# avaneev/avir

Measured on NVIDIA H100. Metric: Mpixels/sec resize (8K->4K RGBA), higher is better.
Workload: dtype f32

## Files before the change

avir_b200/csrc/stream_chain.cu:

```cuda
#include <cuda.h>
#include <cuda_runtime.h>

#include "stream_kernel.cuh"
#include "stream_launch.h"

#if !defined(AVS_CHAIN_ID) || !defined(AVS_CHAIN_PASS)
#error "compile with -DAVS_CHAIN_ID=<StreamChainId> -DAVS_CHAIN_PASS=<0 row pass | 1 column pass>"
#endif

namespace avs {

namespace {

typedef CUresult (*EncodeTiledFn)(CUtensorMap*, CUtensorMapDataType, cuuint32_t, void*, const cuuint64_t*,
                                  const cuuint64_t*, const cuuint32_t*, const cuuint32_t*, CUtensorMapInterleave,
                                  CUtensorMapSwizzle, CUtensorMapL2promotion, CUtensorMapFloatOOBfill);
EncodeTiledFn encode_tiled() {
    static const EncodeTiledFn fn = [] {
        void* f = nullptr;
        cudaDriverEntryPointQueryResult q;
        if (cudaGetDriverEntryPoint("cuTensorMapEncodeTiled", &f, cudaEnableDefault, &q) != cudaSuccess ||
            q != cudaDriverEntryPointSuccess)
            f = nullptr;
        return reinterpret_cast<EncodeTiledFn>(f);
    }();
    return fn;
}

bool encode_source_tensor(StreamParams& p, int box_rows) {
    static_assert(sizeof(CUtensorMap) == sizeof(p.tmap), "tensor map size");
    EncodeTiledFn enc = encode_tiled();
    if (!enc) return false;
    const cuuint64_t dims[2] = {(cuuint64_t)p.n_lines * 4, (cuuint64_t)(p.src_len - p.src_row_base)};
    const cuuint64_t strides[1] = {(cuuint64_t)p.src_pitch * 4};
    const cuuint32_t box[2] = {64, (cuuint32_t)box_rows};
    const cuuint32_t estr[2] = {1, 1};
    if (dims[1] < 1) return false;
    return enc(reinterpret_cast<CUtensorMap*>(p.tmap), CU_TENSOR_MAP_DATA_TYPE_FLOAT32, 2, const_cast<void*>(p.src),
               dims, strides, box, estr, CU_TENSOR_MAP_INTERLEAVE_NONE, CU_TENSOR_MAP_SWIZZLE_NONE,
               CU_TENSOR_MAP_L2_PROMOTION_L2_256B, CU_TENSOR_MAP_FLOAT_OOB_FILL_NONE) == CUDA_SUCCESS;
}

template <class C, bool IS_V, int EPI>
int launch_one(const StreamParams& p_in, int sm_count, cudaStream_t st) {
    StreamParams p = p_in;
    if constexpr (C::MBAR) {
        if (!encode_source_tensor(p, C::SRC_N)) return -3;
    }
    constexpr int NW = IS_V ? C::NWARPS_V : C::NWARPS_H;
    constexpr size_t smem = (size_t)NW * (IS_V ? C::WARP_F2_V : C::WARP_F2_H) * sizeof(float2);
    static_assert(smem <= 227 * 1024, "per-warp rings do not fit the shared memory of an SM");
    auto kern = stream_pass_kernel<C, IS_V, EPI>;
    if (cudaFuncSetAttribute(kern, cudaFuncAttributeMaxDynamicSharedMemorySize, (int)smem) != cudaSuccess)
        return -1;
    const long long rps = (long long)(p.out1 - 1) / C::B - p.out0 / C::B + 1;
    const long long units = rps * stream_strip_count(p);
    long long blocks = (units + NW - 1) / NW;
    if (blocks > sm_count) blocks = sm_count;
    if (blocks < 1) return 0;
    kern<<<(int)blocks, NW * 32, smem, st>>>(p);
    return cudaGetLastError() == cudaSuccess ? 0 : -1;
}

}

template <>
int stream_launch_chain<AVS_CHAIN_ID, (AVS_CHAIN_PASS != 0)>(int variant, int epi, const StreamParams& p, int sm_count,
                                                             void* stream) {
    constexpr bool IS_V = (AVS_CHAIN_PASS != 0);
    cudaStream_t st = static_cast<cudaStream_t>(stream);
    int rc = -2;
    auto run = [&](int var) {
        return stream_dispatch_chain<AVS_CHAIN_ID>(IS_V, var, p.src_type, [&](auto tag, auto pass) {
            using C = typename decltype(tag)::type;
            if constexpr (decltype(pass)::is_v != IS_V) {
                (void)rc;
            } else if constexpr (!IS_V) {
                rc = (p.xs_count != nullptr) ? launch_one<C, false, kEpiXs>(p, sm_count, st)
                                             : launch_one<C, false, 0>(p, sm_count, st);
            } else {
                rc = (epi == 1) ? launch_one<C, true, 1>(p, sm_count, st)
                                : (epi == 2 ? launch_one<C, true, 2>(p, sm_count, st) : launch_one<C, true, 0>(p, sm_count, st));
            }
        });
    };
    bool known = run(variant);
    if (known && rc == -3) known = run(1);
    return known ? rc : -2;
}

}
```

avir_b200/csrc/stream_kernel.cuh:

```cuda
#pragma once

#include <cuda_runtime.h>
#include <stddef.h>
#include <stdint.h>
#include <string.h>

#include "avirb200.h"
#include "pixel_ops.cuh"
#include "stream_types.h"

#if defined(__CUDACC__)
#define AVS_FN __device__ __forceinline__
#define AVS_SYNCWARP() __syncwarp()
#else
#define AVS_FN inline __attribute__((always_inline))
void avs_emul_syncwarp();
#define AVS_SYNCWARP() avs_emul_syncwarp()
#endif

namespace avs {

using avb::lin2srgb;
using avb::round_out;
using avb::round_out_int;
// ... 815 lines not shown
    }
#else
    if (w.lane == 0) {
        const unsigned char* src = static_cast<const unsigned char*>(p.src);
        const size_t rowb = (size_t)p.src_pitch * 4;
        for (int k = 0; k < C::SRC_N; ++k)
            emul_copy(d + k * (kPitchL * 8), src + (size_t)(row + k) * rowb + (size_t)w.line0 * 16, w.nlines * 16);
    }
    (void)bar;
#endif
}

template <class C, bool IS_V, int EPI>
AVS_FN void regwin_round(const StreamParams& p, WarpRun<C, IS_V>& w, RegWin<C>& R, int s1, int s2, int jout) {
    using G = RegWinGeom<C>;
    using S0 = typename C::T0;
    using S1 = typename C::T1;
    using S2 = typename C::T2;
    using R0 = RingOf<C, IS_V, 0>;
    constexpr int OQ = G::Q0 % G::A0;
    const unsigned char* ring0 = reinterpret_cast<const unsigned char*>(w.ring0) + R0::lane_off_b(w.lane);
    const unsigned char* b1 = ring0 + (size_t)s1 * R0::PITCH_B;
    const unsigned char* b2 = ring0 + (size_t)s2 * R0::PITCH_B;
#pragma unroll
    for (int i = 0; i < G::A0; ++i) {
        R.w0[G::Q0 + i] = (i < G::A0 - OQ) ? R0::load(b1 + (OQ + i) * R0::PITCH_B, w.cv)
                                           : R0::load(b2 + (i - (G::A0 - OQ)) * R0::PITCH_B, w.cv);
    }
    float2 o[C::B];
#pragma unroll
    for (int q = 0; q < C::reps0; ++q) {
#pragma unroll
        for (int m = 0; m < S0::M; ++m)
            R.w1[G::K1 + q * S0::M + m] = step_one<S0>(R.w0, q * S0::CH + m * S0::ADV, p.s[0]);
    }
#pragma unroll
    for (int k = 0; k < G::Q0; ++k) R.w0[k] = R.w0[k + G::A0];
#pragma unroll
    for (int q = 0; q < C::reps1; ++q) {
#pragma unroll
        for (int m = 0; m < S1::M; ++m) {
            const float2 v = step_one<S1>(R.w1, q * S1::CH + m * S1::ADV, p.s[1]);
            if constexpr (C::NS == 3) R.w2[G::K2 + q * S1::M + m] = v;
            else o[q * S1::M + m] = v;
        }
    }
#pragma unroll
    for (int k = 0; k < G::K1; ++k) R.w1[k] = R.w1[k + G::A1];
    if constexpr (C::NS == 3) {
#pragma unroll
        for (int q = 0; q < C::reps2; ++q) {
#pragma unroll
            for (int m = 0; m < S2::M; ++m) o[q * S2::M + m] = step_one<S2>(R.w2, q * S2::CH + m * S2::ADV, p.s[2]);
        }
#pragma unroll
        for (int k = 0; k < G::K2; ++k) R.w2[k] = R.w2[k + G::A2];
    }
    constexpr int ML = C::MLAST;
#pragma unroll
    for (int q = 0; q < C::B / ML; ++q) {
        if constexpr (IS_V) {
            sink_v<C, EPI, ML, true>(p, w, jout + q * ML, o + q * ML);
        } else {
            if (q > 0) sink_h_readback<C, ML>(w);
            sink_h_store<C, ML, EPI == kEpiXs>(p, w);
            sink_h_stage<C, ML>(w, jout + q * ML, o + q * ML);
        }
    }
}

template <class C, bool IS_V, int EPI>
AVS_FN void run_regwin(const StreamParams& p, WarpRun<C, IS_V>& w, int r, int n, int groups, int& gslot, int& gi, int& wi) {
    using G = RegWinGeom<C>;
    constexpr int PRO = C::H + C::LOOKAHEAD;
    RegWin<C> R;
    regwin_enter<C, IS_V>(w, R);
    int s1 = w.rd[0] + (G::Q0 / G::A0) * G::A0;
    if (s1 >= C::rsp0) s1 -= C::rsp0;
    int s2 = (s1 + G::A0 == C::rsp0) ? 0 : s1 + G::A0;
    int jout = w.a[C::NS - 1] + C::MLAST * w.kb[C::NS - 1];
    int grow = w.o0 + (r + PRO) * C::SRC_N - p.src_row_base;
    for (int it = n / C::RW_UNROLL; it > 0; --it) {
#pragma unroll
        for (int u = 0; u < C::RW_UNROLL; ++u) {
            if constexpr (C::MBAR) {
                mbar_wait(w.mbar0 + wi * 8, (w.mpar >> wi) & 1u);
                w.mpar ^= 1u << wi;
                wi = (wi + 1 == C::NG) ? 0 : wi + 1;
            } else {
                cp_async_wait<C::LOOKAHEAD - 1>();
            }
            AVS_SYNCWARP();
            if constexpr (!IS_V) sink_h_readback<C, C::MLAST>(w);
            const bool issue = (r + PRO < groups);
            if constexpr (C::MBAR) {
                if (issue) bulk_group<C, IS_V>(p, w, grow, gslot, w.mbar0 + gi * 8);
                grow += C::SRC_N;
                gi = (gi + 1 == C::NG) ? 0 : gi + 1;
            } else {
                load_group<C, IS_V, true>(p, w, r + PRO, gslot, issue);
                cp_async_commit();
            }
            gslot = (gslot + C::SRC_N == C::rsp0) ? 0 : gslot + C::SRC_N;
            regwin_round<C, IS_V, EPI>(p, w, R, s1, s2, jout);
            s1 = s2;
            s2 = (s2 + G::A0 == C::rsp0) ? 0 : s2 + G::A0;
            jout += C::B;
            ++r;
        }
    }
    regwin_leave<C, IS_V>(w, R, n);
}


template <class C, bool IS_V, int EPI>
AVS_FN void run_warp(const StreamParams& p, WarpRun<C, IS_V>& w, int strip, int rho0, int rounds) {
    using S0 = typename C::T0;
    using S1 = typename C::T1;
    using S2 = typename C::T2;
    w.line0 = strip * kLines;
    w.nlines = imin_(kLines, p.n_lines - w.line0);
    if (p.seg_b > 0) {
        const int sa = (p.seg_a + kLines - 1) / kLines;
        if (strip < sa) {
            w.nlines = imin_(kLines, p.seg_a - w.line0);
        } else {
            w.line0 = p.seg_b_line0 + (strip - sa) * kLines;
            w.nlines = imin_(kLines, p.seg_b_line0 + p.seg_b - w.line0);
        }
    }
    if (C::NS == 3) {
        w.a[2] = C::B * rho0;
        w.a[1] = in_first<S2>(p.s[2], w.a[2]);
    } else {
        w.a[1] = C::B * rho0;
    }
    w.a[0] = in_first<S1>(p.s[1], w.a[1]);
    w.o0 = in_first<S0>(p.s[0], w.a[0]);
#pragma unroll
    for (int i = 0; i < kMaxSteps; ++i) w.rd[i] = w.wr[i] = w.kb[i] = 0;

    const int total = rounds + C::DELAY_LAST;
    const int groups = total + C::H;
    const bool fused_rx = IS_V && p.xr_flags != nullptr;
    const int int_lo = fused_rx ? p.xr_own_lo : p.src_lo, int_hi = fused_rx ? p.xr_own_hi : p.src_hi;
    if (fused_rx) {
        const int first = w.o0, last = w.o0 + groups * C::SRC_N;
        if (first < p.xr_own_lo && p.xr_own_lo > p.src_lo) xr_wait(p.xr_flags + 0, p.xr_seq);
        if (last > p.xr_own_hi && p.xr_own_hi < p.src_hi) xr_wait(p.xr_flags + 1, p.xr_seq);
    }
    int gslot = 0;
    int gi = 0, wi = 0;
    constexpr int PRO = C::H + C::LOOKAHEAD;
    loader_init<C, IS_V>(p, w);
    if constexpr (!IS_V) w.pend_j0 = kNoPend;
    if constexpr (!IS_V) {
        w.xs_l0 = w.xs_l1 = w.xs_dir = 0;
        w.xs_delta = 0;
    }
    if constexpr (!IS_V && EPI == kEpiXs) {
        const ptrdiff_t rowb = (ptrdiff_t)p.dst_pitch * 4;
        if (p.xs_up_dst != nullptr && w.line0 < p.xs_top) {
            w.xs_l1 = imin_(w.nlines, p.xs_top - w.line0);
            w.xs_delta = reinterpret_cast<const unsigned char*>(p.xs_up_dst) - static_cast<const unsigned char*>(p.dst);
        } else if (p.xs_dn_dst != nullptr && w.line0 + w.nlines > p.xs_bot0 && w.line0 < p.xs_bot0 + p.xs_bot) {
            w.xs_dir = 1;
            w.xs_l0 = imax_(0, p.xs_bot0 - w.line0);
            w.xs_l1 = imin_(w.nlines, p.xs_bot0 + p.xs_bot - w.line0);
            w.xs_delta = reinterpret_cast<const unsigned char*>(p.xs_dn_dst) - static_cast<const unsigned char*>(p.dst) -
                         (ptrdiff_t)p.xs_bot0 * rowb;
        }
    }
#define AVS_ISSUE_CHECKED(G)                                                                          \
    {                                                                                                 \
        const bool issue_ = (G) < groups;                                                             \
        load_group<C, IS_V, false>(p, w, (G), gslot, issue_);                                         \
        if constexpr (C::MBAR) {                                                                      \
            if (issue_) mbar_arrive_cp_async(w.mbar0 + gi * 8);                                       \
            gi = (gi + 1 == C::NG) ? 0 : gi + 1;                                                      \
        } else {                                                                                      \
            cp_async_commit();                                                                        \
        }                                                                                             \
        gslot = (gslot + C::SRC_N == C::rsp0) ? 0 : gslot + C::SRC_N;                                 \
    }
#define AVS_WAIT_GROUP()                                                                              \
    {                                                                                                 \
        mbar_wait(w.mbar0 + wi * 8, (w.mpar >> wi) & 1u);                                             \
        w.mpar ^= 1u << wi;                                                                           \
        wi = (wi + 1 == C::NG) ? 0 : wi + 1;                                                          \
    }
    for (int g = 0; g < PRO; ++g) AVS_ISSUE_CHECKED(g)
    if constexpr (C::MBAR) {
        for (int g = 0; g < C::H; ++g) AVS_WAIT_GROUP()
    }
    int slo = C::DELAY_LAST, shi = total - 1;
    steady_bounds<C, IS_V, 0, S0>(p, w, C::delay0, C::reps0, slo, shi);
    steady_bounds<C, IS_V, 1, S1>(p, w, C::delay1, C::reps1, slo, shi);
    if constexpr (C::NS == 3) steady_bounds<C, IS_V, 2, S2>(p, w, C::delay2, C::reps2, slo, shi);
    slo = imax_(slo, cdiv_(int_lo - w.o0, C::SRC_N) - PRO);
    {
        const int g_int_hi = fdiv_(int_hi - w.o0, C::SRC_N) - 1;
        if (groups - 1 > g_int_hi) shi = imin_(shi, g_int_hi - PRO);
    }

#define AVS_ROUND(STEADY)                                                                             \
    {                                                                                                 \
        if constexpr (C::MBAR) AVS_WAIT_GROUP()                                                       \
        else cp_async_wait<C::LOOKAHEAD - 1>();  \
        AVS_SYNCWARP();                         \
        if constexpr (STEADY) {                                                                       \
            load_group<C, IS_V, true>(p, w, r + PRO, gslot, r + PRO < groups);                        \
            cp_async_commit();                                                                        \
            gslot = (gslot + C::SRC_N == C::rsp0) ? 0 : gslot + C::SRC_N;                             \
        } else {                                                                                      \
            AVS_ISSUE_CHECKED(r + PRO)                                                                \
        }                                                                                             \
        _Pragma("unroll") for (int q = 0; q < C::reps0; ++q) run_batch<C, IS_V, EPI, 0, S0, STEADY>(p, w); \
        if (STEADY || r >= C::delay1) {                                                               \
            _Pragma("unroll") for (int q = 0; q < C::reps1; ++q) run_batch<C, IS_V, EPI, 1, S1, STEADY>(p, w); \
        }                                                                                             \
        if constexpr (C::NS == 3) {                                                                   \
            if (STEADY || r >= C::delay2) {                                                           \
                _Pragma("unroll") for (int q = 0; q < C::reps2; ++q) run_batch<C, IS_V, EPI, 2, S2, STEADY>(p, w); \
            }                                                                                         \
        }                                                                                             \
    }
    int r = 0;
    while (r < total) {
        if constexpr (C::REGWIN) {
            const int n = (shi - r + 1) / C::RW_UNROLL * C::RW_UNROLL;
            if (r == slo && n > 0) {
                run_regwin<C, IS_V, EPI>(p, w, r, n, groups, gslot, gi, wi);
                r += n;
                continue;
            }
            AVS_ROUND(false)
            ++r;
        } else {
            if (C::STEADY_LOOP && r >= slo && r <= shi) {
                do {
                    AVS_ROUND(true)
                    ++r;
                } while (r <= shi);
            } else {
                AVS_ROUND(false)
                ++r;
            }
        }
    }
#undef AVS_ROUND
#undef AVS_ISSUE_CHECKED
#undef AVS_WAIT_GROUP
    if constexpr (!IS_V) {
        sink_h_readback<C, C::MLAST>(w);
        sink_h_store<C, C::MLAST, EPI == kEpiXs>(p, w);
    }
    if constexpr (!C::MBAR) cp_async_wait<0>();
    AVS_SYNCWARP();
    if constexpr (!IS_V && EPI == kEpiXs) {
        if (w.xs_l1 > w.xs_l0) {
            xs_fence();
            AVS_SYNCWARP();
            if (w.lane == 0) {
                const unsigned long long rps = (unsigned long long)((p.out1 - 1) / C::B - p.out0 / C::B + 1);
                const unsigned long long done = xs_add(p.xs_count + w.xs_dir, (unsigned long long)rounds) + (unsigned long long)rounds;
                if (done == p.xs_units[w.xs_dir] * rps) {
                    p.xs_count[w.xs_dir] = 0;
                    xs_publish(w.xs_dir ? p.xs_dn_flag : p.xs_up_flag, p.xs_seq);
                }
            }
        }
    }
}


template <class C, bool IS_V, int EPI>
AVS_FN void stream_warp_main(const StreamParams& p, long long gw, long long nwarps, int lane, float2* sm,
                             const float* lut) {
    WarpRun<C, IS_V> w;
    w.lane = lane;
    w.cv.lut = lut;
    w.cv.gm = p.in_gamma_mult;
    w.cv.alpha0 = (p.alpha_index == (lane & 1) * 2);
    w.cv.alpha1 = (p.alpha_index == (lane & 1) * 2 + 1);
    w.ring0 = sm;
    w.ring1 = w.ring0 + (IS_V ? (size_t)C::rsp0 * kPitchL : (size_t)C::SRC_RING_F2);
    w.ring2 = w.ring1 + (size_t)C::rsp1 * kPitchL;
    w.stage = w.ring2 + (size_t)C::rsp2 * kPitchL;
    w.mbar0 = 0;
    w.mpar = 0;
    if constexpr (C::MBAR) {
        float2* bars = sm + (IS_V ? C::WARP_F2_V : C::WARP_F2_H) - C::MBAR_F2;
        w.mbar0 = smem_u32(bars);
#if defined(__CUDACC__)
        if (lane == 0) {
            for (int i = 0; i < C::NG; ++i) mbar_init(w.mbar0 + i * 8, 32);
            mbar_init_fence();
        }
        __syncwarp();
#endif
    }
    const int rho_first = p.out0 / C::B, rho_last = (p.out1 - 1) / C::B;
    const int rps = rho_last - rho_first + 1;
    const int nstrips = stream_strip_count(p);
    const long long units = (long long)nstrips * rps;
    long long u0 = gw * units / nwarps;
    const long long u1 = (gw + 1) * units / nwarps;
    while (u0 < u1) {
        const int strip = (int)(u0 / rps);
        const int r0 = (int)(u0 - (long long)strip * rps);
        const long long left = u1 - u0;
        const int rounds = (left < (long long)(rps - r0)) ? (int)left : rps - r0;
        run_warp<C, IS_V, EPI>(p, w, strip, rho_first + r0, rounds);
        u0 += rounds;
    }
}

#if defined(__CUDACC__)
template <class C, bool IS_V, int EPI>
__global__ void __launch_bounds__((IS_V ? C::NWARPS_V : C::NWARPS_H) * 32, 1)
stream_pass_kernel(const __grid_constant__ StreamParams p) {
    constexpr int NW = IS_V ? C::NWARPS_V : C::NWARPS_H;
    constexpr bool SRGB = !IS_V && (C::SRCT == kSrcU8Srgb);
    __shared__ float slut[SRGB ? 256 : 1];
    if constexpr (SRGB) {
        for (int i = threadIdx.x; i < 256; i += NW * 32) slut[i] = __ldg(p.srgb_lut + i);
        __syncthreads();
    }
    extern __shared__ __align__(128) unsigned char stream_smem[];
    const int warp = threadIdx.x >> 5, lane = threadIdx.x & 31;
    float2* sm = reinterpret_cast<float2*>(stream_smem) + (size_t)warp * (IS_V ? C::WARP_F2_V : C::WARP_F2_H);
    stream_warp_main<C, IS_V, EPI>(p, (long long)blockIdx.x * NW + warp, (long long)gridDim.x * NW, lane, sm, slut);
}
#endif



#ifndef AVS_RWU_OVERRIDE
#define AVS_RWU_OVERRIDE 0
#endif
template <class S0, class S1, class S2, int REPS_LAST, int LAH, int LAV, int RWU, int VAR, bool IS_V, int SRCT, int NWMAX = 8>
using ChainV = ChainC<S0, S1, S2, REPS_LAST, (IS_V ? LAV : LAH), (VAR == 2 && !IS_V) ? 1 : VAR, IS_V ? AVIRB200_F32 : SRCT,
                      AVS_RWU_OVERRIDE ? AVS_RWU_OVERRIDE : RWU, NWMAX>;

template <int VAR, bool IS_V, int SRCT = AVIRB200_F32>
using ChainDil24 = ChainV<StepC<K_RESIZE, AVIRB200_SUM_DIL8, 24, 2>, StepC<K_FIR, AVIRB200_SUM_DIL8, 8, 1>, NoStep,
                          1, 2, 3, 1, VAR, IS_V, SRCT>;
template <int VAR, bool IS_V, int SRCT = AVIRB200_F32>
using ChainDil24Q = ChainV<StepC<K_RESIZE, AVIRB200_SUM_DIL8, 24, 2, 4>, StepC<K_FIR, AVIRB200_SUM_DIL8, 8, 1, 4>, NoStep,
                           1, 3, 3, 1, VAR, IS_V, SRCT, 12>;
template <int VAR, bool IS_V, int SRCT = AVIRB200_F32>
using ChainInl24 = ChainV<StepC<K_RESIZE, AVIRB200_SUM_INL, 24, 2>, StepC<K_FIR, AVIRB200_SUM_INL, 7, 1>, NoStep,
                          1, 2, 3, 1, VAR, IS_V, SRCT>;
template <int VAR, bool IS_V, int SRCT = AVIRB200_F32>
using ChainInl3 = ChainV<StepC<K_FIR, AVIRB200_SUM_INL, 7, 1>, StepC<K_RESIZE, AVIRB200_SUM_INL, 18, 2>,
                         StepC<K_FIR, AVIRB200_SUM_INL, 7, 1>, 1, 1, 2, 1, VAR, IS_V, SRCT>;
template <int VAR, bool IS_V, int SRCT = AVIRB200_F32>
using ChainInl3D = ChainV<StepC<K_FIR, AVIRB200_SUM_INL, 15, 2>, StepC<K_RESIZE, AVIRB200_SUM_INL, 18, 2>,
                          StepC<K_FIR, AVIRB200_SUM_INL, 7, 1>, 1, 1, 1, 1, VAR, IS_V, SRCT>;
template <int VAR, bool IS_V, int SRCT = AVIRB200_F32>
using ChainDil56 = ChainV<StepC<K_RESIZE, AVIRB200_SUM_DIL8, 56, 4, 4>, StepC<K_FIR, AVIRB200_SUM_DIL8, 8, 1, 4>, NoStep,
                          1, 1, 1, 1, VAR, IS_V, SRCT>;
template <int VAR, bool IS_V, int SRCT = AVIRB200_F32>
using ChainUp2 = ChainV<StepC<K_FIR, AVIRB200_SUM_INL, 7, 1>, StepC<K_RESIZE2, AVIRB200_SUM_INL, 24, 1>, NoStep,
                        2, 1, 3, 1, VAR, IS_V, SRCT>;

template <class C>
struct ChainTag {
    using type = C;
};

template <bool V>
struct PassTag {
    static constexpr bool is_v = V;
};

template <int ID, class F>
inline bool stream_dispatch_chain(bool is_v, int variant, int src_type, F&& f) {
#define AVS_V(NAME, N)                                                                    \
    case N:                                                                               \
        if (is_v) f(ChainTag<NAME<N, true> >(), PassTag<true>());                         \
        else f(ChainTag<NAME<N, false> >(), PassTag<false>());                            \
        return true;
#if defined(__CUDACC__)
#define AVS_V3(NAME)
#else
#define AVS_V3(NAME) AVS_V(NAME, 3)
#endif
#define AVS_INT_SRC(NAME, T)                                                              \
    if (!is_v && src_type == T) {                                                         \
        if (variant == 0 || variant == 3) f(ChainTag<NAME<0, false, T> >(), PassTag<false>()); \
        else f(ChainTag<NAME<1, false, T> >(), PassTag<false>());                         \
        return true;                                                                      \
    }
#define AVS_VARIANTS(NAME)                                                                \
    AVS_INT_SRC(NAME, AVIRB200_U8)                                                        \
    AVS_INT_SRC(NAME, AVIRB200_U16)                                                       \
    AVS_INT_SRC(NAME, kSrcU8Srgb)                                                         \
    switch (variant) {                                                                    \
        AVS_V(NAME, 0) AVS_V(NAME, 1) AVS_V(NAME, 2) AVS_V3(NAME)                         \
    default: return false;                                                                \
    }
    if (variant < 0 || variant >= kStreamVariants) return false;
    if constexpr (ID == kChainDil24) { AVS_VARIANTS(ChainDil24) }
    else if constexpr (ID == kChainInl24) { AVS_VARIANTS(ChainInl24) }
    else if constexpr (ID == kChainInl3) { AVS_VARIANTS(ChainInl3) }
    else if constexpr (ID == kChainInl3D) { AVS_VARIANTS(ChainInl3D) }
    else if constexpr (ID == kChainDil56) { AVS_VARIANTS(ChainDil56) }
    else if constexpr (ID == kChainUp2) { AVS_VARIANTS(ChainUp2) }
    else if constexpr (ID == kChainDil24Q) { AVS_VARIANTS(ChainDil24Q) }
    else return false;
#undef AVS_VARIANTS
#undef AVS_INT_SRC
#undef AVS_V3
#undef AVS_V
}

template <class F>
inline bool stream_dispatch(int id, bool is_v, int variant, int src_type, F&& f) {
    switch (id) {
    case kChainDil24: return stream_dispatch_chain<kChainDil24>(is_v, variant, src_type, f);
    case kChainInl24: return stream_dispatch_chain<kChainInl24>(is_v, variant, src_type, f);
    case kChainInl3: return stream_dispatch_chain<kChainInl3>(is_v, variant, src_type, f);
    case kChainInl3D: return stream_dispatch_chain<kChainInl3D>(is_v, variant, src_type, f);
    case kChainDil56: return stream_dispatch_chain<kChainDil56>(is_v, variant, src_type, f);
    case kChainUp2: return stream_dispatch_chain<kChainUp2>(is_v, variant, src_type, f);
    case kChainDil24Q: return stream_dispatch_chain<kChainDil24Q>(is_v, variant, src_type, f);
    default: return false;
    }
}

}
```

avir_b200/csrc/stream_types.h:

```cpp
#pragma once

#include <stdint.h>
#include <string.h>

#include "avirb200.h"
#include "device_plan.h"
#include "pass_request.h"

namespace avs {

constexpr int kMaxSteps = 3;
constexpr int kLines = 16;
constexpr int kSrcU8Srgb = 4;
enum { K_FIR = 0, K_RESIZE = 1, K_RESIZE2 = 2, K_NONE = 3 };

constexpr int kTapOne = 64;
struct StreamTap {
    float lo, hi;
};
struct StreamStep {
    int out_len, in_len;
    int edge, latency;
    int sp_first;
    int zero_start;
    StreamTap taps[kTapOne + 1];
};

struct StreamParams {
    StreamStep s[kMaxSteps];
    int n_lines;
    int seg_a, seg_b, seg_b_line0;
    int src_len;
    int out0, out1;
    const void* src;
    int src_type;
    const float* srgb_lut;
    float in_gamma_mult;
    long long src_pitch;
    int src_row_base;
    int src_lo, src_hi;
    void* dst;
    long long dst_pitch;
    int dst_type;
    int dst_row_base;
    int gamma_out, alpha_index;
    float out_gamma_mult;
    int round_mode;
    float tr_mul, tr_mul_inv, pk_out;
    float* xs_up_dst;
    float* xs_dn_dst;
    unsigned* xs_up_flag;
    unsigned* xs_dn_flag;
    unsigned long long* xs_count;
    unsigned long long xs_units[2];
    unsigned xs_seq;
    int xs_top, xs_bot0, xs_bot;
    const float* xr_up_src;
    const float* xr_dn_src;
    const volatile unsigned* xr_flags;
    unsigned xr_seq;
    int xr_own_lo, xr_own_hi;
    alignas(64) unsigned char tmap[128];
};

enum StreamChainId {
    kChainNone = 0,
    kChainDil24,
    kChainInl24,
    kChainInl3,
    kChainInl3D,
    kChainDil56,
    kChainUp2,
    kChainDil24Q,
    kChainCount
};

constexpr int kStreamVariants = 4;
inline int stream_default_variant(int chain, bool is_v) { return (is_v && chain == 5 ) ? 0 : 1; }

struct StreamAxisPlan {
    int chain = kChainNone;
    int nsteps = 0;
    int src_len = 0, dst_len = 0;
    StreamStep s[kMaxSteps];
};

struct StepSpec {
    int kind, sum, nt, adv;
};

inline const StepSpec* chain_spec(int id, int* nsteps) {
    static const StepSpec dil24[] = {{K_RESIZE, AVIRB200_SUM_DIL8, 24, 2}, {K_FIR, AVIRB200_SUM_DIL8, 8, 1}};
    static const StepSpec inl24[] = {{K_RESIZE, AVIRB200_SUM_INL, 24, 2}, {K_FIR, AVIRB200_SUM_INL, 7, 1}};
    static const StepSpec inl3[] = {{K_FIR, AVIRB200_SUM_INL, 7, 1}, {K_RESIZE, AVIRB200_SUM_INL, 18, 2},
                                    {K_FIR, AVIRB200_SUM_INL, 7, 1}};
    static const StepSpec dil56[] = {{K_RESIZE, AVIRB200_SUM_DIL8, 56, 4}, {K_FIR, AVIRB200_SUM_DIL8, 8, 1}};
    static const StepSpec inl3d[] = {{K_FIR, AVIRB200_SUM_INL, 15, 2}, {K_RESIZE, AVIRB200_SUM_INL, 18, 2},
                                     {K_FIR, AVIRB200_SUM_INL, 7, 1}};
    static const StepSpec up2[] = {{K_FIR, AVIRB200_SUM_INL, 7, 1}, {K_RESIZE2, AVIRB200_SUM_INL, 24, 1}};
    switch (id) {
    case kChainDil24: case kChainDil24Q: *nsteps = 2; return dil24;
    case kChainInl24: *nsteps = 2; return inl24;
    case kChainInl3: *nsteps = 3; return inl3;
    case kChainInl3D: *nsteps = 3; return inl3d;
    case kChainDil56: *nsteps = 2; return dil56;
    case kChainUp2: *nsteps = 2; return up2;
    default: *nsteps = 0; return nullptr;
    }
}

inline bool stream_match_step(const avirb200_step_desc& d, const StepSpec& sp, StreamStep& out) {
    memset(&out, 0, sizeof out);
    out.out_len = d.out_len;
    out.in_len = d.in_len;
    out.zero_start = d.zero_start;
    out.taps[kTapOne].lo = out.taps[kTapOne].hi = 1.0f;
    if (sp.kind == K_FIR) {
        if (d.kind != AVIRB200_STEP_FIR || d.ntaps != sp.nt || d.resample != sp.adv) return false;
        if (sp.sum == AVIRB200_SUM_INL && d.ntaps != 2 * d.latency + 1) return false;
        out.edge = d.edge;
        out.latency = d.latency;
        for (int t = 0; t < d.ntaps; ++t) out.taps[t].lo = out.taps[t].hi = d.taps[t];
        return true;
    }
    if (d.kind != AVIRB200_STEP_RESIZE || d.ntaps != sp.nt || d.ntaps > 64 || d.out_len < 1) return false;
    if (sp.kind == K_RESIZE && d.upsampled) return false;
    if (sp.kind == K_RESIZE2 && !(d.upsampled && d.skip_odd)) return false;
    const int step = (sp.kind == K_RESIZE2) ? 1 : sp.adv;
    uint32_t f0 = 0;
    if (d.order) memcpy(&f0, &d.frac[0], 4);
    for (int j = 0; j < d.out_len; ++j) {
        if (d.src_pos[j] != d.src_pos[0] + step * j) return false;
        if (d.phase[j] != d.phase[0]) return false;
        if (d.order) {
            uint32_t fj;
            memcpy(&fj, &d.frac[j], 4);
            if (fj != f0) return false;
        }
    }
    out.sp_first = d.src_pos[0];
    const float* c0 = d.taps + (size_t)d.phase[0] * d.ntaps * (d.order + 1);
    for (int t = 0; t < d.ntaps; ++t) {
        if (d.order) {
            volatile float prod = c0[d.ntaps + t] * d.frac[0];
            out.taps[t].lo = c0[t] + prod;
        } else {
            out.taps[t].lo = c0[t];
        }
        out.taps[t].hi = out.taps[t].lo;
    }
    return true;
}

inline bool stream_plan_axis(const avirb200_axis_desc& ad, int sum_mode, int channels, StreamAxisPlan& out,
                             int allow_deselected = 0, bool is_v = false) {
    out.chain = kChainNone;
    if (channels != 4) return false;
    for (int id = 1; id < kChainCount; ++id) {
        if (id == kChainUp2 && is_v && !allow_deselected) continue;
        if (id == kChainDil24Q && allow_deselected != 2) continue;
        if (id == kChainDil24 && allow_deselected == 2) continue;
        int ns = 0;
        const StepSpec* spec = chain_spec(id, &ns);
        if (ns != ad.nsteps) continue;
        bool ok = true;
        int prev = ad.src_len;
        for (int i = 0; i < ns && ok; ++i) {
            ok = (spec[i].sum == sum_mode) && ad.steps[i].in_len == prev &&
                 stream_match_step(ad.steps[i], spec[i], out.s[i]);
            prev = ad.steps[i].out_len;
        }
        if (!ok || prev != ad.dst_len) continue;
        out.chain = id;
        out.nsteps = ns;
        out.src_len = ad.src_len;
        out.dst_len = ad.dst_len;
        return true;
    }
    return false;
}

inline bool stream_row_source_ok(const avirb200_plan_desc& d) {
    if (d.use_gamma & 1) return d.in_type == AVIRB200_U8;
    return d.in_type == AVIRB200_F32 || d.in_type == AVIRB200_U8 || d.in_type == AVIRB200_U16;
}
#if defined(__CUDACC__)
__host__ __device__
#endif
inline int stream_strip_count(const StreamParams& p) {
    if (p.seg_b > 0) return (p.seg_a + 15) / 16 + (p.seg_b + 15) / 16;
    return (p.n_lines + 15) / 16;
}
inline int stream_epilogue_code(const avirb200_plan_desc& d) {
    if (d.use_gamma & 2) return 0;
    if (d.out_type == AVIRB200_F32) return 1;
    return d.tr_mul == 1.0f ? 2 : 0;
}
inline int stream_row_source_code(const avirb200_plan_desc& d) {
    return (d.use_gamma & 1) ? kSrcU8Srgb : d.in_type;
}

struct StreamMailbox {
    float* from_up = nullptr;
    float* from_dn = nullptr;
    unsigned* flags = nullptr;
    unsigned long long* count = nullptr;
};

struct StreamLink {
    const avirb200_shard_info* me = nullptr;
    const avirb200_shard_info* up = nullptr;
    const avirb200_shard_info* dn = nullptr;
    StreamMailbox mine, above, below;
    unsigned seq = 0;
};
inline int stream_rows_up(const StreamLink& l) { return l.up ? l.up->halo_down : 0; }
inline int stream_rows_down(const StreamLink& l) { return l.dn ? l.dn->halo_up : 0; }

inline bool stream_fused_rx_ok(const StreamLink& l) {
    return (l.up == nullptr || (stream_rows_up(l) > 0) == (l.me->halo_up > 0)) &&
           (l.dn == nullptr || (stream_rows_down(l) > 0) == (l.me->halo_down > 0));
}
inline bool stream_fused_tx_ok(const StreamLink& l) {
    const int top = stream_rows_up(l), bot = stream_rows_down(l);
    return stream_fused_rx_ok(l) && !(top > 0 && bot > 0 && (top + kLines - 1) / kLines > (l.me->src_rows - bot) / kLines);
}

inline void stream_set_sender(StreamParams& p, const StreamLink& l) {
    const int top = stream_rows_up(l), bot = stream_rows_down(l), rows = l.me->src_rows;
    p.xs_seq = l.seq;
    p.xs_count = l.mine.count;
    if (top > 0) {
        p.xs_up_dst = l.above.from_dn;
        p.xs_up_flag = &l.above.flags[1];
        p.xs_top = top;
        p.xs_units[0] = (unsigned long long)((top + kLines - 1) / kLines);
    }
    if (bot > 0) {
        p.xs_dn_dst = l.below.from_up;
        p.xs_dn_flag = &l.below.flags[0];
        p.xs_bot0 = rows - bot;
        p.xs_bot = bot;
        p.xs_units[1] = (unsigned long long)((rows + kLines - 1) / kLines - p.xs_bot0 / kLines);
    }
}

inline void stream_set_receiver(StreamParams& p, const StreamLink& l) {
    p.xr_up_src = l.mine.from_up;
    p.xr_dn_src = l.mine.from_dn;
    p.xr_flags = l.mine.flags;
    p.xr_seq = l.seq;
    p.xr_own_lo = l.me->src_row0;
    p.xr_own_hi = l.me->src_row0 + l.me->src_rows;
}

inline void stream_params(StreamParams& p, const StreamAxisPlan& ap, const avirb200_plan_desc& d,
                          const avb::PassRequest& q, const float* lut) {
    memset(&p, 0, sizeof p);
    for (int i = 0; i < ap.nsteps; ++i) p.s[i] = ap.s[i];
    p.n_lines = q.lines;
    if (q.seg_bot > 0) {
        p.seg_a = q.seg_top;
        p.seg_b = q.seg_bot;
        p.seg_b_line0 = q.lines - q.seg_bot;
    } else if (q.seg_top > 0) {
        p.n_lines = q.seg_top;
    }
    p.src_len = ap.src_len;
    p.out0 = q.out0;
    p.out1 = q.out1;
    p.src = q.src;
    p.src_type = q.is_v ? AVIRB200_F32 : stream_row_source_code(d);
    p.src_pitch = (long long)q.src_pitch;
    p.src_row_base = q.src_base;
    p.src_lo = q.src_lo;
    p.src_hi = q.src_hi;
    p.dst = q.dst;
    p.dst_pitch = (long long)q.dst_pitch;
    p.dst_type = q.dst_type;
    p.dst_row_base = q.dst_base;
    const avb::PixelStage px = avb::pixel_stage(d, lut);
    p.srgb_lut = px.srgb_lut;
    p.in_gamma_mult = px.in_gamma_mult;
    p.gamma_out = px.gamma_out;
    p.alpha_index = px.alpha_index;
    p.out_gamma_mult = px.out_gamma_mult;
    p.round_mode = px.round_mode;
    p.tr_mul = px.tr_mul;
    p.tr_mul_inv = px.tr_mul_inv;
    p.pk_out = px.pk_out;
    if (q.link != nullptr) {
        if (q.is_v) stream_set_receiver(p, *q.link);
        else stream_set_sender(p, *q.link);
    }
}

struct StreamColumns {
    int out0, out1, src_lo, src_hi;
};
inline void stream_fill_row_params(StreamParams& p, const StreamAxisPlan& ap, const avirb200_plan_desc& d,
                                   const void* src, long long src_pitch, float* mid, long long mid_pitch, int rows,
                                   const float* lut, int seg_top = 0, int seg_bot = 0,
                                   const StreamColumns* cols = nullptr) {
    avb::PassRequest q = avb::row_request(d, src, (size_t)src_pitch, rows, mid, (size_t)mid_pitch);
    q.seg_top = seg_top;
    q.seg_bot = seg_bot;
    if (cols != nullptr) {
        q.out0 = q.dst_base = cols->out0;
        q.out1 = cols->out1;
        q.src_base = q.src_lo = cols->src_lo;
        q.src_hi = cols->src_hi;
    }
    stream_params(p, ap, d, q, lut);
}
inline void stream_fill_col_params(StreamParams& p, const StreamAxisPlan& ap, const avirb200_plan_desc& d,
                                   const float* mid, long long mid_pitch, int mid_lo, int mid_hi, void* dst,
                                   long long dst_pitch, int out0, int out1) {
    stream_params(p, ap, d,
                  avb::col_request(d, d.dst_w, mid, (size_t)mid_pitch, mid_lo, mid_hi, dst, (size_t)dst_pitch, out0, out1),
                  nullptr);
}

}
```

Before: 70160.

## Deal column-pass work so each block's warps cover adjacent strips

The column pass no longer splits its strip×row units evenly across all warps. Warps are now grouped into teams whose width is the gcd of warps-per-block and total warps, so each team member handles adjacent strips (grp*width+k) over the same row range. The goal is to make a block's concurrent accesses touch neighbouring memory for better DRAM/L2 locality. The grid size for the column pass is recomputed to match. It also adds a standalone profiling program that compares access patterns, and it risks load imbalance when the strip count is not a multiple of the team width.

```diff
diff --git a/avir_b200/csrc/stream_chain.cu b/avir_b200/csrc/stream_chain.cu
--- a/avir_b200/csrc/stream_chain.cu
+++ b/avir_b200/csrc/stream_chain.cu
@@ -53,10 +53,8 @@
     auto kern = stream_pass_kernel<C, IS_V, EPI>;
     if (cudaFuncSetAttribute(kern, cudaFuncAttributeMaxDynamicSharedMemorySize, (int)smem) != cudaSuccess)
         return -1;
-    const long long rps = (long long)(p.out1 - 1) / C::B - p.out0 / C::B + 1;
-    const long long units = rps * stream_strip_count(p);
-    long long blocks = (units + NW - 1) / NW;
-    if (blocks > sm_count) blocks = sm_count;
+    const int rps = (p.out1 - 1) / C::B - p.out0 / C::B + 1;
+    const long long blocks = stream_blocks(p, IS_V, rps, NW, sm_count);
     if (blocks < 1) return 0;
     kern<<<(int)blocks, NW * 32, smem, st>>>(p);
     return cudaGetLastError() == cudaSuccess ? 0 : -1;
diff --git a/avir_b200/csrc/stream_kernel.cuh b/avir_b200/csrc/stream_kernel.cuh
--- a/avir_b200/csrc/stream_kernel.cuh
+++ b/avir_b200/csrc/stream_kernel.cuh
@@ -1141,18 +1141,10 @@
     }
     const int rho_first = p.out0 / C::B, rho_last = (p.out1 - 1) / C::B;
     const int rps = rho_last - rho_first + 1;
-    const int nstrips = stream_strip_count(p);
-    const long long units = (long long)nstrips * rps;
-    long long u0 = gw * units / nwarps;
-    const long long u1 = (gw + 1) * units / nwarps;
-    while (u0 < u1) {
-        const int strip = (int)(u0 / rps);
-        const int r0 = (int)(u0 - (long long)strip * rps);
-        const long long left = u1 - u0;
-        const int rounds = (left < (long long)(rps - r0)) ? (int)left : rps - r0;
-        run_warp<C, IS_V, EPI>(p, w, strip, rho_first + r0, rounds);
-        u0 += rounds;
-    }
+    const int width = IS_V ? stream_team_width(C::NWARPS_V, nwarps) : 1;
+    StreamDeal deal = stream_deal(stream_strip_count(p), rps, width, gw / width, nwarps / width, (int)(gw % width));
+    StreamRun run;
+    while (stream_next_run<IS_V>(deal, run)) run_warp<C, IS_V, EPI>(p, w, run.strip, rho_first + run.r0, run.rounds);
 }
 
 #if defined(__CUDACC__)
diff --git a/avir_b200/csrc/stream_types.h b/avir_b200/csrc/stream_types.h
--- a/avir_b200/csrc/stream_types.h
+++ b/avir_b200/csrc/stream_types.h
@@ -191,6 +191,60 @@
     if (p.seg_b > 0) return (p.seg_a + 15) / 16 + (p.seg_b + 15) / 16;
     return (p.n_lines + 15) / 16;
 }
+
+#if defined(__CUDACC__)
+__host__ __device__
+#endif
+inline int stream_team_width(int nw, long long nwarps) {
+    long long a = nw, b = nwarps;
+    while (b != 0) {
+        const long long t = a % b;
+        a = b;
+        b = t;
+    }
+    return (int)a;
+}
+struct StreamRun {
+    int strip, r0, rounds;
+};
+struct StreamDeal {
+    long long u, u1;
+    int rps, nstrips, width, k;
+};
+#if defined(__CUDACC__)
+__host__ __device__
+#endif
+inline StreamDeal stream_deal(int nstrips, int rps, int width, long long b, long long nb, int k) {
+    StreamDeal d;
+    const long long units = (long long)((nstrips + width - 1) / width) * rps;
+    d.u = b * units / nb;
+    d.u1 = (b + 1) * units / nb;
+    d.rps = rps;
+    d.nstrips = nstrips;
+    d.width = width;
+    d.k = k;
+    return d;
+}
+template <bool GROUPED>
+#if defined(__CUDACC__)
+__host__ __device__
+#endif
+inline bool stream_next_run(StreamDeal& d, StreamRun& r) {
+    while (d.u < d.u1) {
+        const long long grp = d.u / d.rps;
+        r.r0 = (int)(d.u - grp * d.rps);
+        r.rounds = (d.u1 - d.u < (long long)(d.rps - r.r0)) ? (int)(d.u1 - d.u) : d.rps - r.r0;
+        r.strip = GROUPED ? (int)(grp * d.width) + d.k : (int)grp;
+        d.u += r.rounds;
+        if (!GROUPED || r.strip < d.nstrips) return true;
+    }
+    return false;
+}
+inline long long stream_blocks(const StreamParams& p, bool is_v, int rps, int nw, int sm_count) {
+    const int nstrips = stream_strip_count(p);
+    const long long blocks = is_v ? (long long)((nstrips + nw - 1) / nw) * rps : ((long long)nstrips * rps + nw - 1) / nw;
+    return blocks < sm_count ? blocks : sm_count;
+}
 inline int stream_epilogue_code(const avirb200_plan_desc& d) {
     if (d.use_gamma & 2) return 0;
     if (d.out_type == AVIRB200_F32) return 1;
diff --git a/profiles/access_ceiling.cu b/profiles/access_ceiling.cu
--- /dev/null
+++ b/profiles/access_ceiling.cu
@@ -0,0 +1,256 @@
+#include <cuda_runtime.h>
+
+#include <algorithm>
+#include <cstdio>
+#include <cstdlib>
+#include <string>
+#include <vector>
+
+#define CK(x)                                                                                   \
+    do {                                                                                        \
+        cudaError_t e_ = (x);                                                                   \
+        if (e_ != cudaSuccess) {                                                                \
+            fprintf(stderr, "%s:%d %s: %s\n", __FILE__, __LINE__, #x, cudaGetErrorString(e_)); \
+            exit(1);                                                                            \
+        }                                                                                       \
+    } while (0)
+
+constexpr int SW = 7680, SH = 4320, DW = 3840, DH = 2160;
+constexpr int kNW = 8;
+
+__device__ __forceinline__ void cp16(void* s, const void* g) {
+    const unsigned sa = (unsigned)__cvta_generic_to_shared(s);
+    asm volatile("cp.async.cg.shared.global [%0], [%1], 16;" ::"r"(sa), "l"(g) : "memory");
+}
+__device__ __forceinline__ void commit() { asm volatile("cp.async.commit_group;" ::: "memory"); }
+template <int N>
+__device__ __forceinline__ void wait_groups() { asm volatile("cp.async.wait_group %0;" ::"n"(N) : "memory"); }
+
+constexpr int kColStrips = DW / 16, kColRps = DH / 8, kColLA = 3;
+
+__device__ __forceinline__ void col_run(const float4* src, float4* dst, float4* ring, int lane, int strip, int r0, int n) {
+    const int piece = lane & 15, rsub = lane >> 4;
+    auto issue = [&](int g) {
+        if (g < n) {
+            const int row0 = (r0 + g) * 16;
+            float4* d = ring + (g % (kColLA + 1)) * 256;
+#pragma unroll
+            for (int k = 0; k < 8; ++k)
+                cp16(d + (rsub + 2 * k) * 16 + piece, src + (size_t)(row0 + rsub + 2 * k) * DW + strip * 16 + piece);
+        }
+        commit();
+    };
+    for (int g = 0; g < kColLA; ++g) issue(g);
+    const int q = lane >> 1, c = lane & 1;
+    for (int r = 0; r < n; ++r) {
+        issue(r + kColLA);
+        wait_groups<kColLA>();
+        __syncwarp();
+        const float2* s = reinterpret_cast<const float2*>(ring + (r % (kColLA + 1)) * 256);
+        float2* o = reinterpret_cast<float2*>(dst + (size_t)(r0 + r) * 8 * DW + strip * 16) + lane;
+#pragma unroll
+        for (int m = 0; m < 8; ++m) o[(size_t)m * DW * 2] = s[(2 * m) * 32 + q * 2 + c];
+        __syncwarp();
+    }
+    wait_groups<0>();
+    __syncwarp();
+}
+
+__global__ void __launch_bounds__(kNW * 32, 1) col_a(const float4* src, float4* dst) {
+    extern __shared__ float4 sm[];
+    const int warp = threadIdx.x >> 5, lane = threadIdx.x & 31;
+    float4* ring = sm + warp * (kColLA + 1) * 256;
+    const long long units = (long long)kColStrips * kColRps, nw = (long long)gridDim.x * kNW, gw = blockIdx.x * kNW + warp;
+    long long u0 = gw * units / nw;
+    const long long u1 = (gw + 1) * units / nw;
+    while (u0 < u1) {
+        const int strip = (int)(u0 / kColRps), r0 = (int)(u0 % kColRps);
+        const int n = (int)(u1 - u0 < kColRps - r0 ? u1 - u0 : kColRps - r0);
+        col_run(src, dst, ring, lane, strip, r0, n);
+        u0 += n;
+    }
+}
+
+__global__ void __launch_bounds__(kNW * 32, 1) col_b(const float4* src, float4* dst) {
+    extern __shared__ float4 sm[];
+    const int warp = threadIdx.x >> 5, lane = threadIdx.x & 31;
+    float4* ring = sm + warp * (kColLA + 1) * 256;
+    const long long units = (long long)(kColStrips / kNW) * kColRps;
+    long long u0 = blockIdx.x * units / gridDim.x;
+    const long long u1 = (blockIdx.x + 1) * units / gridDim.x;
+    while (u0 < u1) {
+        const int grp = (int)(u0 / kColRps), r0 = (int)(u0 % kColRps);
+        const int n = (int)(u1 - u0 < kColRps - r0 ? u1 - u0 : kColRps - r0);
+        col_run(src, dst, ring, lane, grp * kNW + warp, r0, n);
+        u0 += n;
+    }
+}
+
+constexpr int kRowStrips = SH / 16, kRowRps = DW / 8;
+
+template <int F, int D>
+__device__ __forceinline__ void row_run(const float4* src, float4* dst, float4* ring, int lane, int strip, int r0, int n) {
+    const int pos = lane & 15, lsub = lane >> 4;
+    const int nf = (n + F - 1) / F;
+    auto issue = [&](int f) {
+        if (f < nf) {
+            float4* d = ring + (f % (D + 1)) * (F * 256);
+#pragma unroll
+            for (int g = 0; g < F; ++g) {
+                const int p = (r0 + f * F + g) * 16 + pos;
+                if (f * F + g < n) {
+#pragma unroll
+                    for (int k = 0; k < 8; ++k)
+                        cp16(d + (lsub + 2 * k) * (F * 16) + g * 16 + pos, src + (size_t)(strip * 16 + lsub + 2 * k) * SW + p);
+                }
+            }
+        }
+        commit();
+    };
+    for (int f = 0; f < D; ++f) issue(f);
+    const int opos = lane & 7, osub = lane >> 3;
+    for (int f = 0; f < nf; ++f) {
+        issue(f + D);
+        wait_groups<D>();
+        __syncwarp();
+        const float4* s = ring + (f % (D + 1)) * (F * 256);
+#pragma unroll
+        for (int g = 0; g < F; ++g) {
+            const int r = f * F + g;
+            if (r < n) {
+                float4* o = dst + (size_t)(strip * 16 + osub) * DW + (r0 + r) * 8 + opos;
+#pragma unroll
+                for (int k = 0; k < 4; ++k) o[(size_t)4 * k * DW] = s[(osub + 4 * k) * (F * 16) + g * 16 + 2 * opos];
+            }
+        }
+        __syncwarp();
+    }
+    wait_groups<0>();
+    __syncwarp();
+}
+
+template <int F, int D>
+__global__ void __launch_bounds__(kNW * 32, 1) row_a(const float4* src, float4* dst, int nwb) {
+    extern __shared__ float4 sm[];
+    const int warp = threadIdx.x >> 5, lane = threadIdx.x & 31;
+    if (warp >= nwb) return;
+    float4* ring = sm + warp * (D + 1) * F * 256;
+    const long long units = (long long)kRowStrips * kRowRps, nw = (long long)gridDim.x * nwb, gw = blockIdx.x * nwb + warp;
+    long long u0 = gw * units / nw;
+    const long long u1 = (gw + 1) * units / nw;
+    while (u0 < u1) {
+        const int strip = (int)(u0 / kRowRps), r0 = (int)(u0 % kRowRps);
+        const int n = (int)(u1 - u0 < kRowRps - r0 ? u1 - u0 : kRowRps - r0);
+        row_run<F, D>(src, dst, ring, lane, strip, r0, n);
+        u0 += n;
+    }
+}
+
+__global__ void __launch_bounds__(kNW * 32, 1) copy_d(const float4* __restrict__ src, float4* __restrict__ dst, size_t n_out) {
+    const size_t stride = (size_t)gridDim.x * blockDim.x;
+    for (size_t i = (size_t)blockIdx.x * blockDim.x + threadIdx.x; i < n_out; i += 4 * stride) {
+        float4 a[4], b[4];
+#pragma unroll
+        for (int u = 0; u < 4; ++u) {
+            const size_t j = i + u * stride;
+            if (j < n_out) {
+                a[u] = __ldcs(src + j);
+                b[u] = __ldcs(src + n_out + j);
+            }
+        }
+#pragma unroll
+        for (int u = 0; u < 4; ++u) {
+            const size_t j = i + u * stride;
+            if (j < n_out) __stcs(dst + j, make_float4(a[u].x, b[u].y, a[u].z, b[u].w));
+        }
+    }
+}
+
+__global__ void flush_kernel(float4* p, size_t n, float v) {
+    for (size_t i = (size_t)blockIdx.x * blockDim.x + threadIdx.x; i < n; i += (size_t)gridDim.x * blockDim.x)
+        p[i] = make_float4(v, v, v, v);
+}
+
+int main(int argc, char** argv) {
+    const int reps = argc > 1 ? atoi(argv[1]) : 30;
+    cudaDeviceProp prop;
+    CK(cudaGetDeviceProperties(&prop, 0));
+    const int sms = prop.multiProcessorCount;
+    const size_t n_src = (size_t)SW * SH, n_mid = (size_t)DW * SH, n_dst = (size_t)DW * DH, n_flush = (size_t)64 << 20;
+    float4 *src, *mid, *dst, *fl;
+    CK(cudaMalloc(&src, n_src * 16));
+    CK(cudaMalloc(&mid, n_mid * 16));
+    CK(cudaMalloc(&dst, n_dst * 16));
+    CK(cudaMalloc(&fl, n_flush * 16));
+    CK(cudaMemset(src, 0, n_src * 16));
+    CK(cudaMemset(mid, 0, n_mid * 16));
+
+    struct Pat {
+        std::string name;
+        double bytes;
+        int smem;
+        void (*launch)(int, int, const float4*, float4*, const float4*, float4*, float4*);
+    };
+    const double row_b = (double)(n_src + n_mid) * 16, col_b_ = (double)(n_mid + n_dst) * 16;
+    auto set_smem = [](const void* k, int b) { CK(cudaFuncSetAttribute(k, cudaFuncAttributeMaxDynamicSharedMemorySize, b)); };
+    const int col_sm = kNW * (kColLA + 1) * 256 * 16;
+    set_smem((const void*)col_a, col_sm);
+    set_smem((const void*)col_b, col_sm);
+    const int row1 = kNW * 3 * 256 * 16, row2 = kNW * 2 * 2 * 256 * 16, row4_w = (227 * 1024) / (2 * 4 * 256 * 16);
+    const int row4 = row4_w * 2 * 4 * 256 * 16;
+    set_smem((const void*)row_a<1, 2>, row1);
+    set_smem((const void*)row_a<2, 1>, row2);
+    set_smem((const void*)row_a<4, 1>, row4);
+    std::vector<Pat> pats = {
+        {"col a  strip-major units, 256-B pieces", col_b_, col_sm,
+         [](int sms, int sm, const float4*, float4*, const float4* m, float4* d, float4*) { col_a<<<sms, kNW * 32, sm>>>(m, d); }},
+        {"col b  8 adjacent strips per block", col_b_, col_sm,
+         [](int sms, int sm, const float4*, float4*, const float4* m, float4* d, float4*) { col_b<<<sms, kNW * 32, sm>>>(m, d); }},
+        {"col d  contiguous copy", col_b_, 0,
+         [](int sms, int, const float4*, float4*, const float4* m, float4* d, float4*) {
+             copy_d<<<sms, kNW * 32>>>(m, d, (size_t)DW * DH);
+         }},
+        {"row a  256-B fetches per line, 2 in flight", row_b, row1,
+         [](int sms, int sm, const float4* s, float4* m, const float4*, float4*, float4*) { row_a<1, 2><<<sms, kNW * 32, sm>>>(s, m, kNW); }},
+        {"row c2 512-B fetches per line, 1 in flight", row_b, row2,
+         [](int sms, int sm, const float4* s, float4* m, const float4*, float4*, float4*) { row_a<2, 1><<<sms, kNW * 32, sm>>>(s, m, kNW); }},
+        {"row c4 1-KB fetches per line, 1 in flight, " + std::to_string(row4_w) + " warps", row_b, row4,
+         [](int sms, int sm, const float4* s, float4* m, const float4*, float4*, float4*) {
+             row_a<4, 1><<<sms, kNW * 32, sm>>>(s, m, (227 * 1024) / (2 * 4 * 256 * 16));
+         }},
+        {"row d  contiguous copy", row_b, 0,
+         [](int sms, int, const float4* s, float4* m, const float4*, float4*, float4*) {
+             copy_d<<<sms, kNW * 32>>>(s, m, (size_t)DW * SH);
+         }},
+    };
+    cudaEvent_t e0, e1;
+    CK(cudaEventCreate(&e0));
+    CK(cudaEventCreate(&e1));
+    std::vector<std::vector<float>> t(pats.size());
+    for (int rep = -2; rep < reps; ++rep) {
+        for (size_t i = 0; i < pats.size(); ++i) {
+            flush_kernel<<<sms * 4, 256>>>(fl, n_flush, (float)rep);
+            CK(cudaEventRecord(e0));
+            pats[i].launch(sms, pats[i].smem, src, mid, mid, dst, fl);
+            CK(cudaEventRecord(e1));
+            CK(cudaEventSynchronize(e1));
+            CK(cudaGetLastError());
+            float ms = 0;
+            CK(cudaEventElapsedTime(&ms, e0, e1));
+            if (rep >= 0) t[i].push_back(ms);
+        }
+    }
+    printf("device %s, %d SMs; median of %d launches each, patterns alternated, L2 flushed before every launch\n",
+           prop.name, sms, reps);
+    printf("%-48s %9s %9s %9s %8s\n", "pattern", "MB", "ms", "GB/s", "of d");
+    for (size_t i = 0; i < pats.size(); ++i) {
+        std::sort(t[i].begin(), t[i].end());
+        const double med = t[i][t[i].size() / 2];
+        const size_t dref = (i < 3) ? 2 : 6;
+        std::sort(t[dref].begin(), t[dref].end());
+        const double dmed = t[dref][t[dref].size() / 2];
+        printf("%-48s %9.1f %9.4f %9.1f %8.3f   (min %.4f max %.4f)\n", pats[i].name.c_str(), pats[i].bytes / 1e6, med,
+               pats[i].bytes / med / 1e6, dmed / med, t[i].front(), t[i].back());
+    }
+    return 0;
+}
diff --git a/profiles/access_ceiling.py b/profiles/access_ceiling.py
--- /dev/null
+++ b/profiles/access_ceiling.py
@@ -0,0 +1,39 @@
+import argparse
+import os
+import shutil
+import subprocess
+import sys
+import tempfile
+
+HERE = os.path.dirname(os.path.abspath(__file__))
+
+
+def nvcc():
+    for c in (os.environ.get("CUDA_HOME", "") + "/bin/nvcc", "/usr/local/cuda/bin/nvcc", shutil.which("nvcc") or ""):
+        if c and os.path.exists(c):
+            return c
+    sys.exit("nvcc not found")
+
+
+def main():
+    ap = argparse.ArgumentParser()
+    ap.add_argument("--reps", type=int, default=30, help="timed launches per pattern (median reported)")
+    ap.add_argument("--out", help="also write the report here")
+    a = ap.parse_args()
+    with tempfile.TemporaryDirectory() as tmp:
+        exe = os.path.join(tmp, "access_ceiling")
+        subprocess.run([nvcc(), "-O3", "-std=c++17", "-gencode", "arch=compute_90a,code=sm_90a",
+                        os.path.join(HERE, "access_ceiling.cu"), "-o", exe], check=True)
+        card = subprocess.run(["nvidia-smi", "--id=0", "--query-gpu=name,power.limit,clocks.max.sm",
+                               "--format=csv,noheader"], capture_output=True, text=True).stdout.strip()
+        run = subprocess.run([exe, str(a.reps)], capture_output=True, text=True)
+    report = "card: %s\n%s%s" % (card, run.stdout, run.stderr)
+    print(report, end="")
+    if a.out:
+        with open(a.out, "w") as f:
+            f.write(report)
+    sys.exit(run.returncode)
+
+
+if __name__ == "__main__":
+    main()
```

Result: no change. 70810 (median of 6 runs) (+0.9%).
